# georgeretsi/smirk

Measured on NVIDIA H100. Metric: faces/sec encode->FLAME->render @224^2, higher is better.
Workload: dtype tf32x3

## Files before the change

smirk_b200/csrc/xdw_tc.cu:

```cuda
#include "gemm_tc.cuh"
#include "xdw_tc.cuh"
#include "tc_ptx.cuh"

namespace smk {
namespace {

constexpr int BKB = 128, BK = 32, MMA_K = 8;
constexpr int WIN = 16;
constexpr int HALF_BYTES = 128 * BKB;
constexpr int KB_BYTES = 2 * HALF_BYTES;
constexpr int NC = 32;
constexpr int B_BYTES = NC * BKB;
constexpr int E_PITCH = NC + 4;
constexpr int E_FLOATS = 256 * E_PITCH, E_BYTES = E_FLOATS * 4;
constexpr int PAR_ROWS = 13;
constexpr int PAR_FLOATS = PAR_ROWS * NC, PAR_SLOT_BYTES = PAR_FLOATS * 4;
constexpr int NUM_WORKERS = 256;
constexpr int NUM_THREADS = NUM_WORKERS + 32;
constexpr int DW_THREADS = 128, DW_ROLES = NUM_WORKERS / DW_THREADS, WS_THREADS = NUM_WORKERS + DW_THREADS + 128;
constexpr int WS_LAUNCH_REGS = 65536 / WS_THREADS, MMA_REGS = 168, DW_REGS = 136, PROD_REGS = 40;
static_assert(NUM_WORKERS * MMA_REGS + DW_THREADS * DW_REGS + 128 * PROD_REGS == 65536, "register budgets of the pipelined schedule");
static_assert(MMA_REGS >= WS_LAUNCH_REGS && DW_REGS >= WS_LAUNCH_REGS && PROD_REGS <= WS_LAUNCH_REGS,
              "setmaxnreg directions: inc for the MMA and depthwise warpgroups, dec for the producer");
constexpr int MAX_NKB = 5;
constexpr int SMEM_PER_SM = 228 * 1024, SMEM_PER_CTA = 227 * 1024, SMEM_RESERVED = 1024;

template <int NKB, int X3> struct XdwSmem {
    static constexpr int WIN_BYTES = NKB * KB_BYTES;
    static constexpr int STAGE_BYTES = X3 ? 2 * B_BYTES : B_BYTES;
    static constexpr size_t bytes(int wbuf, int stages, int ne) {
        return (size_t)wbuf * WIN_BYTES + stages * STAGE_BYTES + ne * E_BYTES + (X3 ? ne : 2) * PAR_SLOT_BYTES + 256 + 1024;
    }
    static constexpr bool fits(int wbuf, int stages, int ne, int minb) {
        return bytes(wbuf, stages, ne) <= SMEM_PER_CTA && minb * (bytes(wbuf, stages, ne) + SMEM_RESERVED) <= SMEM_PER_SM;
    }
    static constexpr int MINB = !X3 && fits(1, 2, 1, 2) ? 2 : 1;
    static constexpr int NE = X3 && fits(1, 2, 2, 1) ? 2 : 1;
    static constexpr int STAGES = NKB > 2 && fits(1, NKB, NE, MINB) ? NKB : 2;
    static constexpr int WBUF = fits(2, STAGES, NE, MINB) ? 2 : 1;
    static constexpr size_t SMEM = bytes(WBUF, STAGES, NE);
    static constexpr int RING = WBUF * WIN_BYTES, E_OFF = RING + STAGES * STAGE_BYTES, PAR_OFF = E_OFF + NE * E_BYTES,
                         BAR_OFF = PAR_OFF + (X3 ? NE : 2) * PAR_SLOT_BYTES;
    static_assert(fits(WBUF, STAGES, NE, MINB), "shared-memory budget");
    static_assert(2 * (STAGES + WBUF + NE) * 8 <= 256, "barrier block");
};
static_assert(XdwSmem<1, 2>::NE == 2 && XdwSmem<2, 2>::NE == 2 && XdwSmem<3, 2>::NE == 2 && XdwSmem<4, 2>::NE == 2,
              "3xTF32: two E slots for every window the encoder launches (Cin <= 112)");

using namespace ptx;
__device__ __forceinline__ void worker_barrier() { named_barrier(1, NUM_WORKERS); }

struct XdwMaps { CUtensorMap x[2], w[2], wlo[2]; };

struct XdwArgs {
    int H, W, Ho, Wo;
    int mid, nchunks;
    int groups, chunks_per_group;
    int n_items, B;
    int d_grp, d_tx, d_ty, d_img;
    unsigned geom;
    int pad;
    int tiles_x, tiles_y;
    const float* scale1[2]; const float* bias1[2];
    const float* wdw[2];
    const float* scale2[2]; const float* bias2[2];
    float* out[2];
    int round_out;
    float* e_out[2];
};

struct Item { int prob, img, oh0, ow0, c_begin, c_end; };
struct ItemIter {
    int item, grp, tx, ty, img2;
    __device__ explicit ItemIter(const XdwArgs& a) {
        int v = item = blockIdx.x;
        grp = v % a.groups; v /= a.groups; tx = v % a.tiles_x; v /= a.tiles_x; ty = v % a.tiles_y; img2 = v / a.tiles_y;
    }
    __device__ void next(const XdwArgs& a) {
        item += gridDim.x;
        grp += a.d_grp; if (grp >= a.groups) { grp -= a.groups; ++tx; }
        tx += a.d_tx;   if (tx >= a.tiles_x) { tx -= a.tiles_x; ++ty; }
        ty += a.d_ty;   if (ty >= a.tiles_y) { ty -= a.tiles_y; ++img2; }
        img2 += a.d_img;
    }
    template <int TO> __device__ Item decode(const XdwArgs& a) const {
        Item w;
        w.prob = img2 >= a.B ? 1 : 0; w.img = img2 - w.prob * a.B;
        w.oh0 = ty * TO; w.ow0 = tx * TO;
        w.c_begin = grp * a.chunks_per_group; w.c_end = min(a.nchunks, w.c_begin + a.chunks_per_group);
        return w;
    }
};

template <int STRIDE, int X3, int NKB>
__device__ __forceinline__ void produce(const XdwMaps& mp, const XdwArgs& a, uint8_t* smem, uint64_t* full, uint64_t* empty,
                                        uint64_t* wfull, uint64_t* wempty) {
    using L = XdwSmem<NKB, X3>;
    constexpr int TO = STRIDE == 1 ? 14 : 7, STAGES = L::STAGES, WBUF = L::WBUF;
    uint8_t* ring = smem + L::RING;
    int it = 0, n = 0;
    for (ItemIter ii(a); ii.item < a.n_items; ii.next(a), ++n) {
        const Item w = ii.decode<TO>(a);
        const int ey0 = w.oh0 * STRIDE - a.pad, ex0 = w.ow0 * STRIDE - a.pad;
        const int b = n % WBUF;
        mbar_wait(&wempty[b], ((uint32_t)(n / WBUF) & 1u) ^ 1u);
        uint8_t* win = smem + b * L::WIN_BYTES;
        mbar_expect_tx(&wfull[b], (uint32_t)L::WIN_BYTES);
#pragma unroll
        for (int kb = 0; kb < NKB; ++kb) {
            tma_load_4d(&mp.x[w.prob], win + kb * KB_BYTES, &wfull[b], kb * BK, ex0, ey0, w.img);
            tma_load_4d(&mp.x[w.prob], win + kb * KB_BYTES + HALF_BYTES, &wfull[b], kb * BK, ex0, ey0 + 8, w.img);
        }
        for (int c = w.c_begin; c < w.c_end; ++c)
            for (int kb = 0; kb < NKB; ++kb, ++it) {
                const int s = it % STAGES;
                mbar_wait(&empty[s], ((uint32_t)(it / STAGES) & 1u) ^ 1u);
                uint8_t* st = ring + s * L::STAGE_BYTES;
                mbar_expect_tx(&full[s], (uint32_t)L::STAGE_BYTES);
                tma_load_2d(&mp.w[w.prob], st, &full[s], kb * BK, c * NC);
                if (X3) tma_load_2d(&mp.wlo[w.prob], st + B_BYTES, &full[s], kb * BK, c * NC);
            }
    }
}

struct ParLoader {
    const float* src[2];
    int prow, pcol;
    bool owner;
    __device__ ParLoader(const XdwArgs& a, int t) : src{nullptr, nullptr}, prow(t >> 4), pcol((t & 15) * 2), owner(t < PAR_ROWS * 16) {
        if (owner) {
#pragma unroll
            for (int q = 0; q < 2; ++q)
                src[q] = (prow == 0 ? a.scale1[q] : prow == 1 ? a.bias1[q] : prow == 11 ? a.scale2[q] : prow == 12 ? a.bias2[q]
                                                                                  : a.wdw[q] + (size_t)(prow - 2) * a.mid) + pcol;
        }
    }
    __device__ float2 load(const XdwArgs& a, int prob, int c) const {
        float2 v = make_float2(0.f, 0.f);
        if (owner && c * NC + pcol < a.mid) v = __ldg(reinterpret_cast<const float2*>(src[prob] + c * NC));
        return v;
    }
    __device__ void park(float* par, const float2& v) const {
        if (owner) *reinterpret_cast<float2*>(par + prow * NC + pcol) = v;
    }
};

template <int X3, int NKB, int KSL>
__device__ __forceinline__ void expand_gemm(float (&acc)[2][NC / 2], const uint8_t* win, uint8_t* ring, uint64_t* full, uint64_t* empty,
                                            int& it, int wq, int lane) {
    using L = XdwSmem<NKB, X3>;
    constexpr int STAGES = L::STAGES;
#pragma unroll
    for (int mb = 0; mb < 2; ++mb)
#pragma unroll
        for (int i = 0; i < NC / 2; ++i) acc[mb][i] = 0.f;
#pragma unroll
    for (int kb = 0; kb < NKB; ++kb, ++it) {
        const int nks = kb + 1 < NKB ? BK / MMA_K : KSL;
        const int s = it % STAGES;
        mbar_wait(&full[s], (uint32_t)(it / STAGES) & 1u);
        const uint8_t* xa = win + kb * KB_BYTES;
        const uint32_t sb = smem_u32(ring + s * L::STAGE_BYTES);
        if constexpr (X3 != 0) {
            uint32_t hi[2][BK / MMA_K][4], lo[2][BK / MMA_K][4];
#pragma unroll
            for (int mb = 0; mb < 2; ++mb)
#pragma unroll
                for (int k = 0; k < nks; ++k) {
                    float v[4];
                    load_a_frag(xa, mb * 64, k * MMA_K, wq, lane, v);
                    split_frag(v, hi[mb][k], lo[mb][k]);
                }
            wgmma_fence();
#pragma unroll
            for (int k = 0; k < nks; ++k) {
                const uint64_t db = make_smem_desc(sb + k * MMA_K * 4);
                const uint64_t dbl = make_smem_desc(sb + B_BYTES + k * MMA_K * 4);
#pragma unroll
                for (int mb = 0; mb < 2; ++mb) {
                    Wgmma<NC>::rs(acc[mb], hi[mb][k], db, 1u);
                    Wgmma<NC>::rs(acc[mb], lo[mb][k], db, 1u);
                    Wgmma<NC>::rs(acc[mb], hi[mb][k], dbl, 1u);
                }
            }
        } else {
            const uint32_t sa = smem_u32(xa);
            wgmma_fence();
#pragma unroll
            for (int k = 0; k < nks; ++k) {
                const uint64_t db = make_smem_desc(sb + k * MMA_K * 4);
#pragma unroll
                for (int mb = 0; mb < 2; ++mb)
                    Wgmma<NC>::ss(acc[mb], make_smem_desc(sa + mb * 64 * BKB + k * MMA_K * 4), db, 1u);
            }
        }
        wgmma_commit();
        wgmma_wait<0>();
        __syncwarp();
        mbar_arrive_if(&empty[s], lane == 0);
    }
}

template <int STRIDE, bool SAVE>
__device__ __forceinline__ void bn1_relu(const float (&acc)[2][NC / 2], float* E, const float* par, const XdwArgs& a, const Item& w,
                                         int ch0, int half, int wq, int lane) {
    constexpr int TO = STRIDE == 1 ? 14 : 7;
    const int ey0 = w.oh0 * STRIDE - a.pad, ex0 = w.ow0 * STRIDE - a.pad;
#pragma unroll
    for (int mb = 0; mb < 2; ++mb)
#pragma unroll
        for (int hr = 0; hr < 2; ++hr) {
            const int r = mb * 64 + wq * 16 + (lane >> 2) + 8 * hr;
            const int ey = ey0 + half * 8 + (r >> 4), ex = ex0 + (r & 15);
            const bool inside = ey >= 0 && ey < a.H && ex >= 0 && ex < a.W;
            float* erow = E + (size_t)(half * 128 + r) * E_PITCH;
            bool own = false;
            float* esave = nullptr;
            if constexpr (SAVE) {
                own = inside && ey >= w.oh0 * STRIDE && ey < (w.oh0 + TO) * STRIDE && ex >= w.ow0 * STRIDE && ex < (w.ow0 + TO) * STRIDE;
                esave = a.e_out[w.prob] + (((size_t)w.img * a.H + ey) * a.W + ex) * a.mid + ch0;
            }
#pragma unroll
            for (int j = 0; j < NC / 8; ++j) {
                const int ch = 8 * j + 2 * (lane & 3);
                float2 o = make_float2(0.f, 0.f);
                if (inside) {
                    const float2 sc = *reinterpret_cast<const float2*>(par + ch);
                    const float2 bi = *reinterpret_cast<const float2*>(par + NC + ch);
                    o.x = fmaxf(fmaf(acc[mb][4 * j + 2 * hr], sc.x, bi.x), 0.f);
                    o.y = fmaxf(fmaf(acc[mb][4 * j + 2 * hr + 1], sc.y, bi.y), 0.f);
                }
                *reinterpret_cast<float2*>(erow + ch) = o;
                if (SAVE && own && ch0 + ch < a.mid) *reinterpret_cast<float2*>(esave + ch) = o;
            }
        }
}

template <int TO> __device__ __forceinline__ unsigned dw_role(const XdwArgs& a, int slot) {
    const int ncols_e = a.Wo - (a.tiles_x - 1) * TO;
    return (unsigned)(slot % TO) | (unsigned)(slot / TO) << 8 | (unsigned)(slot % ncols_e) << 16 | (unsigned)(slot / ncols_e) << 24;
}
struct DwRows { int ox, oy0, oy1; };
template <int TO> __device__ __forceinline__ DwRows dw_rows(const XdwArgs& a, const ItemIter& ii, unsigned role) {
    const bool col_e = ii.tx == a.tiles_x - 1, row_e = ii.ty == a.tiles_y - 1;
    const int nrows = row_e ? a.Ho - (a.tiles_y - 1) * TO : TO;
    const unsigned g8 = a.geom >> ((col_e ? 16 : 0) + (row_e ? 8 : 0));
    const int rpt = (int)(g8 & 15u), n_rg = (int)((g8 >> 4) & 15u);
    const unsigned r16 = role >> (col_e ? 16 : 0);
    const int rg = (int)((r16 >> 8) & 255u);
    DwRows d;
    d.ox = (int)(r16 & 255u); d.oy0 = rg * rpt; d.oy1 = rg < n_rg ? min(nrows, d.oy0 + rpt) : 0;
    return d;
}

template <int STRIDE>
__device__ __forceinline__ void depthwise(const float* E, const float* par, const XdwArgs& a, const Item& w, int ch0, int cq, const DwRows& rows) {
    if (cq * 4 < a.mid - ch0 && rows.oy0 < rows.oy1) {
        const int ch = ch0 + cq * 4;
        float4 k[9];
#pragma unroll
        for (int q = 0; q < 9; ++q) k[q] = *reinterpret_cast<const float4*>(par + (2 + q) * NC + cq * 4);
        const float4 s2 = *reinterpret_cast<const float4*>(par + 11 * NC + cq * 4);
        const float4 b2 = *reinterpret_cast<const float4*>(par + 12 * NC + cq * 4);
        float* orow = a.out[w.prob] + (((size_t)w.img * a.Ho + w.oh0 + rows.oy0) * a.Wo + w.ow0 + rows.ox) * a.mid + ch;
        const size_t orow_stride = (size_t)a.Wo * a.mid;
        auto emit = [&](const float4& acc4) {
            float4 o = fma4(acc4, s2, b2);
            o.x = fmaxf(o.x, 0.f); o.y = fmaxf(o.y, 0.f); o.z = fmaxf(o.z, 0.f); o.w = fmaxf(o.w, 0.f);
            if (a.round_out) { o.x = round_tf32(o.x); o.y = round_tf32(o.y); o.z = round_tf32(o.z); o.w = round_tf32(o.w); }
            *reinterpret_cast<float4*>(orow) = o;
            orow += orow_stride;
        };
        const float* e = E + (size_t)((rows.oy0 * STRIDE) * WIN + rows.ox * STRIDE) * E_PITCH + cq * 4;
        const float4 zero = make_float4(0.f, 0.f, 0.f, 0.f);
        if (STRIDE == 1) {
            float4 acc0 = zero, acc1 = zero, acc2 = zero;
            const int n_in = rows.oy1 - rows.oy0 + 2;
#pragma unroll 3
            for (int r = 0; r < n_in; ++r, e += WIN * E_PITCH) {
                const float4 x0 = *reinterpret_cast<const float4*>(e);
                const float4 x1 = *reinterpret_cast<const float4*>(e + E_PITCH);
                const float4 x2 = *reinterpret_cast<const float4*>(e + 2 * E_PITCH);
                fma4_acc(acc0, x0, k[6]); fma4_acc(acc0, x1, k[7]); fma4_acc(acc0, x2, k[8]);
                fma4_acc(acc1, x0, k[3]); fma4_acc(acc1, x1, k[4]); fma4_acc(acc1, x2, k[5]);
                fma4_acc(acc2, x0, k[0]); fma4_acc(acc2, x1, k[1]); fma4_acc(acc2, x2, k[2]);
                if (r >= 2) emit(acc0);
                acc0 = acc1; acc1 = acc2; acc2 = zero;
            }
        } else {
            float4 p0 = *reinterpret_cast<const float4*>(e);
            float4 p1 = *reinterpret_cast<const float4*>(e + E_PITCH);
            float4 p2 = *reinterpret_cast<const float4*>(e + 2 * E_PITCH);
            for (int oy = rows.oy0; oy < rows.oy1; ++oy) {
                e += WIN * E_PITCH;
                float4 acc4 = zero;
                fma4_acc(acc4, p0, k[0]); fma4_acc(acc4, p1, k[1]); fma4_acc(acc4, p2, k[2]);
                const float4 m0 = *reinterpret_cast<const float4*>(e);
                const float4 m1 = *reinterpret_cast<const float4*>(e + E_PITCH);
                const float4 m2 = *reinterpret_cast<const float4*>(e + 2 * E_PITCH);
                fma4_acc(acc4, m0, k[3]); fma4_acc(acc4, m1, k[4]); fma4_acc(acc4, m2, k[5]);
                e += WIN * E_PITCH;
                p0 = *reinterpret_cast<const float4*>(e);
                p1 = *reinterpret_cast<const float4*>(e + E_PITCH);
                p2 = *reinterpret_cast<const float4*>(e + 2 * E_PITCH);
                fma4_acc(acc4, p0, k[6]); fma4_acc(acc4, p1, k[7]); fma4_acc(acc4, p2, k[8]);
                emit(acc4);
            }
        }
    }
}

template <int NKB, int X3> struct XdwShared {
    using L = XdwSmem<NKB, X3>;
    uint8_t* smem;
    float* E;
    float* PAR;
    uint64_t *full, *empty;
    uint64_t *wfull, *wempty;
    uint64_t *efull, *eempty;
    __device__ explicit XdwShared(uint8_t* raw) {
        smem = raw + ((1024u - (smem_u32(raw) & 1023u)) & 1023u);
        E = reinterpret_cast<float*>(smem + L::E_OFF);
        PAR = reinterpret_cast<float*>(smem + L::PAR_OFF);
        full = reinterpret_cast<uint64_t*>(smem + L::BAR_OFF);
        empty = full + L::STAGES;
        wfull = empty + L::STAGES;
        wempty = wfull + L::WBUF;
        efull = wempty + L::WBUF;
        eempty = efull + L::NE;
    }
};

template <int STRIDE, int X3, int NKB, int KSL, bool SAVE>
__global__ void __launch_bounds__(NUM_THREADS, XdwSmem<NKB, X3>::MINB)
xdw_kernel(const __grid_constant__ XdwMaps mp, const XdwArgs a) {
    using L = XdwSmem<NKB, X3>;
    constexpr int TO = STRIDE == 1 ? 14 : 7;
    extern __shared__ uint8_t smem_raw[];
    const XdwShared<NKB, X3> sh(smem_raw);
    const int warp = threadIdx.x >> 5, lane = threadIdx.x & 31;
    if (warp == NUM_WORKERS / 32 && lane == 0) {
        prefetch_tensormap(&mp.x[0]);
        prefetch_tensormap(&mp.w[0]);
        for (int s = 0; s < L::STAGES; ++s) { mbar_init(&sh.full[s], 1); mbar_init(&sh.empty[s], NUM_WORKERS / 32); }
        for (int b = 0; b < L::WBUF; ++b) { mbar_init(&sh.wfull[b], 1); mbar_init(&sh.wempty[b], NUM_WORKERS / 32); }
        fence_barrier_init();
    }
    __syncthreads();

    if (warp == NUM_WORKERS / 32) {
        if (lane == 0) produce<STRIDE, X3, NKB>(mp, a, sh.smem, sh.full, sh.empty, sh.wfull, sh.wempty);
        return;
    }

    const int half = warp >> 2, wq = warp & 3;
    const int t = threadIdx.x;
    const int cq = t & 7;
    const ParLoader pl(a, t);
    ItemIter ii(a);
    if (ii.item < a.n_items) { const Item w0 = ii.decode<TO>(a); pl.park(sh.PAR, pl.load(a, w0.prob, w0.c_begin)); }
    worker_barrier();
    const unsigned role = dw_role<TO>(a, t >> 3);
    int cc = 0, it = 0;
    for (int n = 0; ii.item < a.n_items; ++n) {
      const Item w = ii.decode<TO>(a);
      const int wb = n % L::WBUF;
      const uint8_t* win = sh.smem + wb * L::WIN_BYTES + half * HALF_BYTES;
      mbar_wait(&sh.wfull[wb], (uint32_t)(n / L::WBUF) & 1u);
      const DwRows rows = dw_rows<TO>(a, ii, role);
      int next_first = -1, next_prob = 0;
      ii.next(a);
      if (ii.item < a.n_items) { const Item wn = ii.decode<TO>(a); next_first = wn.c_begin; next_prob = wn.prob; }
      for (int c = w.c_begin; c < w.c_end; ++c, ++cc) {
        const int buf = cc & 1;
        const float* par = sh.PAR + buf * PAR_FLOATS;
        const int c_next = c + 1 < w.c_end ? c + 1 : next_first;
        float2 pf = make_float2(0.f, 0.f);
        if (c_next >= 0) pf = pl.load(a, c + 1 < w.c_end ? w.prob : next_prob, c_next);
        float acc[2][NC / 2];
        expand_gemm<X3, NKB, KSL>(acc, win, sh.smem + L::RING, sh.full, sh.empty, it, wq, lane);
        mbar_arrive_if(&sh.wempty[wb], lane == 0 && c + 1 == w.c_end);
        bn1_relu<STRIDE, SAVE>(acc, sh.E, par, a, w, c * NC, half, wq, lane);
        if (c_next >= 0) pl.park(sh.PAR + (buf ^ 1) * PAR_FLOATS, pf);
        worker_barrier();
        depthwise<STRIDE>(sh.E, par, a, w, c * NC, cq, rows);
        worker_barrier();
      }
    }
}

template <int STRIDE, int X3, int NKB, int KSL, bool SAVE>
__global__ void __launch_bounds__(WS_THREADS, 1)
xdw_ws_kernel(const __grid_constant__ XdwMaps mp, const XdwArgs a) {
    using L = XdwSmem<NKB, X3>;
    constexpr int TO = STRIDE == 1 ? 14 : 7, NE = L::NE;
    constexpr int PROD_WARP = (NUM_WORKERS + DW_THREADS) / 32;
    extern __shared__ uint8_t smem_raw[];
    const XdwShared<NKB, X3> sh(smem_raw);
    const int warp = threadIdx.x >> 5, lane = threadIdx.x & 31;
    if (warp == PROD_WARP && lane == 0) {
        prefetch_tensormap(&mp.x[0]);
        prefetch_tensormap(&mp.w[0]);
        prefetch_tensormap(&mp.wlo[0]);
        for (int s = 0; s < L::STAGES; ++s) { mbar_init(&sh.full[s], 1); mbar_init(&sh.empty[s], NUM_WORKERS / 32); }
        for (int b = 0; b < L::WBUF; ++b) { mbar_init(&sh.wfull[b], 1); mbar_init(&sh.wempty[b], NUM_WORKERS / 32); }
        for (int s = 0; s < NE; ++s) { mbar_init(&sh.efull[s], NUM_WORKERS); mbar_init(&sh.eempty[s], DW_THREADS); }
        fence_barrier_init();
    }
    __syncthreads();

    if (warp >= PROD_WARP) {
        setmaxnreg_dec<PROD_REGS>();
        if (warp == PROD_WARP && lane == 0) produce<STRIDE, X3, NKB>(mp, a, sh.smem, sh.full, sh.empty, sh.wfull, sh.wempty);
        return;
    }

    if (warp >= NUM_WORKERS / 32) {
        setmaxnreg_inc<DW_REGS>();
        const int d = threadIdx.x - NUM_WORKERS, cq = d & 7;
        unsigned role[DW_ROLES];
#pragma unroll
        for (int j = 0; j < DW_ROLES; ++j) role[j] = dw_role<TO>(a, (d >> 3) + j * (DW_THREADS / 8));
        int cc = 0;
        for (ItemIter ii(a); ii.item < a.n_items; ii.next(a)) {
            const Item w = ii.decode<TO>(a);
            DwRows rows[DW_ROLES];
#pragma unroll
            for (int j = 0; j < DW_ROLES; ++j) rows[j] = dw_rows<TO>(a, ii, role[j]);
            for (int c = w.c_begin; c < w.c_end; ++c, ++cc) {
                const int s = cc % NE;
                mbar_wait(&sh.efull[s], (uint32_t)(cc / NE) & 1u);
#pragma unroll 1
                for (int j = 0; j < DW_ROLES; ++j) depthwise<STRIDE>(sh.E + s * E_FLOATS, sh.PAR + s * PAR_FLOATS, a, w, c * NC, cq, rows[j]);
                mbar_arrive(&sh.eempty[s]);
            }
        }
        return;
    }

    setmaxnreg_inc<MMA_REGS>();
    const int half = warp >> 2, wq = warp & 3;
    const ParLoader pl(a, threadIdx.x);
    int cc = 0, it = 0, n = 0;
    for (ItemIter ii(a); ii.item < a.n_items; ii.next(a), ++n) {
        const Item w = ii.decode<TO>(a);
        const int wb = n % L::WBUF;
        const uint8_t* win = sh.smem + wb * L::WIN_BYTES + half * HALF_BYTES;
        mbar_wait(&sh.wfull[wb], (uint32_t)(n / L::WBUF) & 1u);
        for (int c = w.c_begin; c < w.c_end; ++c, ++cc) {
            const int s = cc % NE;
            float* par = sh.PAR + s * PAR_FLOATS;
            const float2 pf = pl.load(a, w.prob, c);
            float acc[2][NC / 2];
            expand_gemm<X3, NKB, KSL>(acc, win, sh.smem + L::RING, sh.full, sh.empty, it, wq, lane);
            mbar_arrive_if(&sh.wempty[wb], lane == 0 && c + 1 == w.c_end);
            mbar_wait(&sh.eempty[s], ((uint32_t)(cc / NE) & 1u) ^ 1u);
            pl.park(par, pf);
            worker_barrier();
            bn1_relu<STRIDE, SAVE>(acc, sh.E + s * E_FLOATS, par, a, w, c * NC, half, wq, lane);
            mbar_arrive(&sh.efull[s]);
        }
    }
}

template <int STRIDE, int X3, int NKB, int KSL, bool SAVE>
int launch(const XdwMaps& mp, const XdwArgs& a, int grid, cudaStream_t st) {
    constexpr size_t smem = XdwSmem<NKB, X3>::SMEM;
    if constexpr (X3 != 0) {
        SMK_CHECK_CUDA((set_max_dynamic_smem<xdw_ws_kernel<STRIDE, X3, NKB, KSL, SAVE>>((int)smem)));
        SMK_LAUNCH((xdw_ws_kernel<STRIDE, X3, NKB, KSL, SAVE>), dim3(grid), dim3(WS_THREADS), smem, st, mp, a);
    } else {
        SMK_CHECK_CUDA((set_max_dynamic_smem<xdw_kernel<STRIDE, X3, NKB, KSL, SAVE>>((int)smem)));
        SMK_LAUNCH((xdw_kernel<STRIDE, X3, NKB, KSL, SAVE>), dim3(grid), dim3(NUM_THREADS), smem, st, mp, a);
    }
    SMK_CHECK_LAUNCH();
    return 0;
}

template <int STRIDE, int X3, int NKB, int KSL>
int launch_save(const XdwMaps& mp, const XdwArgs& a, int grid, cudaStream_t st) {
    return a.e_out[0] ? launch<STRIDE, X3, NKB, KSL, true>(mp, a, grid, st) : launch<STRIDE, X3, NKB, KSL, false>(mp, a, grid, st);
}

template <int STRIDE, int X3, int NKB>
int launch_ksl(int ksl, const XdwMaps& mp, const XdwArgs& a, int grid, cudaStream_t st) {
    switch (ksl) {
        case 1: return launch_save<STRIDE, X3, NKB, 1>(mp, a, grid, st);
        case 2: return launch_save<STRIDE, X3, NKB, 2>(mp, a, grid, st);
        case 3: return launch_save<STRIDE, X3, NKB, 3>(mp, a, grid, st);
        default: return launch_save<STRIDE, X3, NKB, 4>(mp, a, grid, st);
    }
}

template <int STRIDE, int X3>
int launch_cin(int Cin, const XdwMaps& mp, const XdwArgs& a, int grid, cudaStream_t st) {
    static_assert(MAX_NKB == 5, "one case per window size");
    const int nkb = cdiv(Cin, BK), ksl = cdiv(Cin, MMA_K) - (nkb - 1) * (BK / MMA_K);
    switch (nkb) {
        case 1: return launch_ksl<STRIDE, X3, 1>(ksl, mp, a, grid, st);
        case 2: return launch_ksl<STRIDE, X3, 2>(ksl, mp, a, grid, st);
        case 3: return launch_ksl<STRIDE, X3, 3>(ksl, mp, a, grid, st);
        case 4: return launch_ksl<STRIDE, X3, 4>(ksl, mp, a, grid, st);
        default: return launch_ksl<STRIDE, X3, 5>(ksl, mp, a, grid, st);
    }
}

}

int xdw_conv(const XdwConv& p, cudaStream_t st, const XdwConv* p2) {
    const int nprob = p2 ? 2 : 1;
    SMK_REQUIRE(p.stride == 1 || p.stride == 2, "xdw_conv: stride must be 1 or 2");
    SMK_REQUIRE(p.Cin % 4 == 0 && p.mid % 4 == 0, "xdw_conv: Cin and mid must be multiples of 4");
    SMK_REQUIRE(p.Cin > 0 && p.Cin <= MAX_NKB * BK, "xdw_conv: Cin must be at most 160 (the whole input window stays in shared memory)");
    SMK_REQUIRE(p.stride == 1 || (p.H % 2 == 0 && p.W % 2 == 0), "xdw_conv: stride 2 expects even input sizes (TF-SAME pad_begin 0)");
    SMK_REQUIRE(!p2 || (p2->B == p.B && p2->H == p.H && p2->W == p.W && p2->Cin == p.Cin && p2->mid == p.mid && p2->stride == p.stride &&
                        p2->round_out == p.round_out && !p2->w1t_lo == !p.w1t_lo && !p2->e_out == !p.e_out),
                "xdw_conv: paired problems must have identical shapes");
    const int Ho = (p.H + p.stride - 1) / p.stride, Wo = (p.W + p.stride - 1) / p.stride;
    const int TO = p.stride == 1 ? 14 : 7;
    XdwMaps mp;
    XdwArgs a{};
    for (int g = 0; g < nprob; ++g) {
        const XdwConv& q = g ? *p2 : p;
        if (int rc = encode_nhwc(&mp.x[g], q.x, q.B, q.H, q.W, q.Cin, q.Cin, WIN, 8, "xdw_conv(x)")) return rc;
        if (int rc = encode_2d(&mp.w[g], q.w1t, (uint64_t)q.mid, (uint64_t)q.Cin, (uint64_t)q.Cin, NC, "xdw_conv(w1)")) return rc;
        mp.wlo[g] = mp.w[g];
        if (q.w1t_lo) { if (int rc = encode_2d(&mp.wlo[g], q.w1t_lo, (uint64_t)q.mid, (uint64_t)q.Cin, (uint64_t)q.Cin, NC, "xdw_conv(w1 tails)")) return rc; }
        a.scale1[g] = q.scale1; a.bias1[g] = q.bias1; a.wdw[g] = q.wdw; a.scale2[g] = q.scale2; a.bias2[g] = q.bias2; a.out[g] = q.out;
        a.e_out[g] = q.e_out;
    }
    if (nprob == 1) {
        mp.x[1] = mp.x[0]; mp.w[1] = mp.w[0]; mp.wlo[1] = mp.wlo[0];
        a.scale1[1] = a.scale1[0]; a.bias1[1] = a.bias1[0]; a.wdw[1] = a.wdw[0]; a.scale2[1] = a.scale2[0]; a.bias2[1] = a.bias2[0]; a.out[1] = a.out[0];
        a.e_out[1] = a.e_out[0];
    }
    const int slots = num_sms();
    a.H = p.H; a.W = p.W; a.Ho = Ho; a.Wo = Wo; a.mid = p.mid; a.nchunks = cdiv(p.mid, NC);
    {
        const long tiles = (long)nprob * cdiv(Wo, TO) * cdiv(Ho, TO) * p.B;
        int groups = (int)std::min<long>(a.nchunks, std::max<long>(1, (slots + tiles - 1) / tiles));
        a.chunks_per_group = cdiv(a.nchunks, groups);
        a.groups = cdiv(a.nchunks, a.chunks_per_group);
    }
    a.pad = p.stride == 1 ? 1 : 0;
    a.tiles_x = cdiv(Wo, TO); a.tiles_y = cdiv(Ho, TO);
    a.round_out = p.round_out;
    {
        const double px_in = (double)nprob * p.B * p.H * p.W, px_out = (double)nprob * p.B * Ho * Wo;
        const char* tag = p.w1t_lo ? "xdw_fused_tc3x" : "xdw_fused_tc";
        if (g_prof_detail) tag = prof_shape_tag(tag, (long)px_out, p.Cin, p.mid);
        SMK_TAG(tag, 4.0 * (px_in * p.Cin + px_out * p.mid + (double)nprob * p.mid * (p.Cin + 13)), 2.0 * px_in * p.Cin * p.mid + 18.0 * px_out * p.mid, st);
    }
    a.B = p.B;
    a.n_items = nprob * a.tiles_x * a.tiles_y * p.B * a.groups;
    {
        const int ncols_e = Wo - (a.tiles_x - 1) * TO, nrows_e = Ho - (a.tiles_y - 1) * TO;
        auto group = [](int ncols, int nrows) { const int n_rg = std::min(32 / ncols, nrows); return (unsigned)((nrows + n_rg - 1) / n_rg) | (unsigned)n_rg << 4; };
        a.geom = group(TO, TO) | group(TO, nrows_e) << 8 | group(ncols_e, TO) << 16 | group(ncols_e, nrows_e) << 24;
    }
    const int grid = std::min(a.n_items, slots);
    { int v = grid; a.d_grp = v % a.groups; v /= a.groups; a.d_tx = v % a.tiles_x; v /= a.tiles_x; a.d_ty = v % a.tiles_y; a.d_img = v / a.tiles_y; }
    if (p.w1t_lo) return p.stride == 1 ? launch_cin<1, 2>(p.Cin, mp, a, grid, st) : launch_cin<2, 2>(p.Cin, mp, a, grid, st);
    return p.stride == 1 ? launch_cin<1, 0>(p.Cin, mp, a, grid, st) : launch_cin<2, 0>(p.Cin, mp, a, grid, st);
}

}

extern "C" int smk_debug_xdw(const float* x, int B, int H, int W, int Cin, const float* w1t, const float* scale1, const float* bias1,
                             int mid, const float* wdw, const float* scale2, const float* bias2, int stride, int round_out,
                             float* out, void* stream) {
    smk::XdwConv p{};
    p.x = x; p.B = B; p.H = H; p.W = W; p.Cin = Cin; p.w1t = w1t; p.scale1 = scale1; p.bias1 = bias1; p.mid = mid; p.wdw = wdw;
    p.scale2 = scale2; p.bias2 = bias2; p.stride = stride; p.round_out = round_out; p.out = out;
    return smk::xdw_conv(p, (cudaStream_t)stream);
}

extern "C" int smk_debug_xdw3x(const float* x, int B, int H, int W, int Cin, const float* w1t_hi, const float* w1t_lo, const float* scale1,
                               const float* bias1, int mid, const float* wdw, const float* scale2, const float* bias2, int stride,
                               float* out, void* stream) {
    smk::XdwConv p{};
    p.x = x; p.B = B; p.H = H; p.W = W; p.Cin = Cin; p.w1t = w1t_hi; p.w1t_lo = w1t_lo; p.scale1 = scale1; p.bias1 = bias1; p.mid = mid; p.wdw = wdw;
    p.scale2 = scale2; p.bias2 = bias2; p.stride = stride; p.round_out = 0; p.out = out;
    return smk::xdw_conv(p, (cudaStream_t)stream);
}
```

Measured before the change: 26320.

## Move BN param staging to depthwise warpgroup and compute two columns per role

```diff
diff --git a/smirk_b200/csrc/xdw_tc.cu b/smirk_b200/csrc/xdw_tc.cu
--- a/smirk_b200/csrc/xdw_tc.cu
+++ b/smirk_b200/csrc/xdw_tc.cu
@@ -17,7 +17,7 @@
 constexpr int PAR_FLOATS = PAR_ROWS * NC, PAR_SLOT_BYTES = PAR_FLOATS * 4;
 constexpr int NUM_WORKERS = 256;
 constexpr int NUM_THREADS = NUM_WORKERS + 32;
-constexpr int DW_THREADS = 128, DW_ROLES = NUM_WORKERS / DW_THREADS, WS_THREADS = NUM_WORKERS + DW_THREADS + 128;
+constexpr int DW_THREADS = 128, WS_THREADS = NUM_WORKERS + DW_THREADS + 128;
 constexpr int WS_LAUNCH_REGS = 65536 / WS_THREADS, MMA_REGS = 168, DW_REGS = 136, PROD_REGS = 40;
 static_assert(NUM_WORKERS * MMA_REGS + DW_THREADS * DW_REGS + 128 * PROD_REGS == 65536, "register budgets of the pipelined schedule");
 static_assert(MMA_REGS >= WS_LAUNCH_REGS && DW_REGS >= WS_LAUNCH_REGS && PROD_REGS <= WS_LAUNCH_REGS,
@@ -29,7 +29,7 @@
     static constexpr int WIN_BYTES = NKB * KB_BYTES;
     static constexpr int STAGE_BYTES = X3 ? 2 * B_BYTES : B_BYTES;
     static constexpr size_t bytes(int wbuf, int stages, int ne) {
-        return (size_t)wbuf * WIN_BYTES + stages * STAGE_BYTES + ne * E_BYTES + (X3 ? ne : 2) * PAR_SLOT_BYTES + 256 + 1024;
+        return (size_t)wbuf * WIN_BYTES + stages * STAGE_BYTES + ne * E_BYTES + (X3 ? 2 * ne : 2) * PAR_SLOT_BYTES + 256 + 1024;
     }
     static constexpr bool fits(int wbuf, int stages, int ne, int minb) {
         return bytes(wbuf, stages, ne) <= SMEM_PER_CTA && minb * (bytes(wbuf, stages, ne) + SMEM_RESERVED) <= SMEM_PER_SM;
@@ -40,7 +40,7 @@
     static constexpr int WBUF = fits(2, STAGES, NE, MINB) ? 2 : 1;
     static constexpr size_t SMEM = bytes(WBUF, STAGES, NE);
     static constexpr int RING = WBUF * WIN_BYTES, E_OFF = RING + STAGES * STAGE_BYTES, PAR_OFF = E_OFF + NE * E_BYTES,
-                         BAR_OFF = PAR_OFF + (X3 ? NE : 2) * PAR_SLOT_BYTES;
+                         BAR_OFF = PAR_OFF + (X3 ? 2 * NE : 2) * PAR_SLOT_BYTES;
     static_assert(fits(WBUF, STAGES, NE, MINB), "shared-memory budget");
     static_assert(2 * (STAGES + WBUF + NE) * 8 <= 256, "barrier block");
 };
@@ -91,6 +91,18 @@
         return w;
     }
 };
+template <int TO> struct ChunkIter {
+    ItemIter ii;
+    int prob, c, c_end;
+    __device__ explicit ChunkIter(const XdwArgs& a) : ii(a) { start(a); }
+    __device__ bool valid(const XdwArgs& a) const { return ii.item < a.n_items; }
+    __device__ void start(const XdwArgs& a) {
+        if (valid(a)) { const Item w = ii.decode<TO>(a); prob = w.prob; c = w.c_begin; c_end = w.c_end; }
+    }
+    __device__ void next(const XdwArgs& a) {
+        if (valid(a) && ++c == c_end) { ii.next(a); start(a); }
+    }
+};
 
 template <int STRIDE, int X3, int NKB>
 __device__ __forceinline__ void produce(const XdwMaps& mp, const XdwArgs& a, uint8_t* smem, uint64_t* full, uint64_t* empty,
@@ -135,9 +147,9 @@
                                                                                   : a.wdw[q] + (size_t)(prow - 2) * a.mid) + pcol;
         }
     }
-    __device__ float2 load(const XdwArgs& a, int prob, int c) const {
+    template <bool SELECT = false> __device__ float2 load(const XdwArgs& a, int prob, int c) const {
         float2 v = make_float2(0.f, 0.f);
-        if (owner && c * NC + pcol < a.mid) v = __ldg(reinterpret_cast<const float2*>(src[prob] + c * NC));
+        if (owner && c * NC + pcol < a.mid) v = __ldg(reinterpret_cast<const float2*>((SELECT ? (prob ? src[1] : src[0]) : src[prob]) + c * NC));
         return v;
     }
     __device__ void park(float* par, const float2& v) const {
@@ -236,25 +248,30 @@
         }
 }
 
-template <int TO> __device__ __forceinline__ unsigned dw_role(const XdwArgs& a, int slot) {
-    const int ncols_e = a.Wo - (a.tiles_x - 1) * TO;
-    return (unsigned)(slot % TO) | (unsigned)(slot / TO) << 8 | (unsigned)(slot % ncols_e) << 16 | (unsigned)(slot / ncols_e) << 24;
-}
-struct DwRows { int ox, oy0, oy1; };
-template <int TO> __device__ __forceinline__ DwRows dw_rows(const XdwArgs& a, const ItemIter& ii, unsigned role) {
+__host__ __device__ constexpr int dw_cols(int stride, bool pipelined) { return stride == 1 && pipelined ? 2 : 1; }
+template <int STRIDE, int DWC> __device__ __forceinline__ unsigned dw_role(const XdwArgs& a, int slot) {
+    constexpr int TO = STRIDE == 1 ? 14 : 7, NCR = (TO + DWC - 1) / DWC;
+    const int ncr_e = (a.Wo - (a.tiles_x - 1) * TO + DWC - 1) / DWC;
+    return (unsigned)(slot % NCR * DWC) | (unsigned)(slot / NCR) << 8 | (unsigned)(slot % ncr_e * DWC) << 16 | (unsigned)(slot / ncr_e) << 24;
+}
+struct DwRows { int ox, ncol, oy0, oy1; };
+template <int STRIDE, int DWC> __device__ __forceinline__ DwRows dw_rows(const XdwArgs& a, const ItemIter& ii, unsigned role) {
+    constexpr int TO = STRIDE == 1 ? 14 : 7;
     const bool col_e = ii.tx == a.tiles_x - 1, row_e = ii.ty == a.tiles_y - 1;
-    const int nrows = row_e ? a.Ho - (a.tiles_y - 1) * TO : TO;
+    const int nrows = row_e ? a.Ho - (a.tiles_y - 1) * TO : TO, ncols = col_e ? a.Wo - (a.tiles_x - 1) * TO : TO;
     const unsigned g8 = a.geom >> ((col_e ? 16 : 0) + (row_e ? 8 : 0));
     const int rpt = (int)(g8 & 15u), n_rg = (int)((g8 >> 4) & 15u);
     const unsigned r16 = role >> (col_e ? 16 : 0);
     const int rg = (int)((r16 >> 8) & 255u);
     DwRows d;
-    d.ox = (int)(r16 & 255u); d.oy0 = rg * rpt; d.oy1 = rg < n_rg ? min(nrows, d.oy0 + rpt) : 0;
+    d.ox = (int)(r16 & 255u); d.ncol = min(DWC, ncols - d.ox);
+    d.oy0 = rg * rpt; d.oy1 = rg < n_rg ? min(nrows, d.oy0 + rpt) : 0;
     return d;
 }
 
-template <int STRIDE>
+template <int STRIDE, int DWC>
 __device__ __forceinline__ void depthwise(const float* E, const float* par, const XdwArgs& a, const Item& w, int ch0, int cq, const DwRows& rows) {
+    static_assert(STRIDE == 1 || DWC == 1, "stride 2 runs one column per role");
     if (cq * 4 < a.mid - ch0 && rows.oy0 < rows.oy1) {
         const int ch = ch0 + cq * 4;
         float4 k[9];
@@ -264,16 +281,19 @@
         const float4 b2 = *reinterpret_cast<const float4*>(par + 12 * NC + cq * 4);
         float* orow = a.out[w.prob] + (((size_t)w.img * a.Ho + w.oh0 + rows.oy0) * a.Wo + w.ow0 + rows.ox) * a.mid + ch;
         const size_t orow_stride = (size_t)a.Wo * a.mid;
-        auto emit = [&](const float4& acc4) {
+        auto bn2 = [&](const float4& acc4) {
             float4 o = fma4(acc4, s2, b2);
             o.x = fmaxf(o.x, 0.f); o.y = fmaxf(o.y, 0.f); o.z = fmaxf(o.z, 0.f); o.w = fmaxf(o.w, 0.f);
             if (a.round_out) { o.x = round_tf32(o.x); o.y = round_tf32(o.y); o.z = round_tf32(o.z); o.w = round_tf32(o.w); }
-            *reinterpret_cast<float4*>(orow) = o;
+            return o;
+        };
+        auto emit = [&](const float4& acc4) {
+            *reinterpret_cast<float4*>(orow) = bn2(acc4);
             orow += orow_stride;
         };
         const float* e = E + (size_t)((rows.oy0 * STRIDE) * WIN + rows.ox * STRIDE) * E_PITCH + cq * 4;
         const float4 zero = make_float4(0.f, 0.f, 0.f, 0.f);
-        if (STRIDE == 1) {
+        if (STRIDE == 1 && DWC == 1) {
             float4 acc0 = zero, acc1 = zero, acc2 = zero;
             const int n_in = rows.oy1 - rows.oy0 + 2;
 #pragma unroll 3
@@ -287,6 +307,45 @@
                 if (r >= 2) emit(acc0);
                 acc0 = acc1; acc1 = acc2; acc2 = zero;
             }
+        } else if (STRIDE == 1) {
+            struct Acc { float4 c[DWC]; };
+            float4 x[DWC + 2];
+            auto load = [&](int r) {
+#pragma unroll
+                for (int j = 0; j < DWC + 2; ++j) x[j] = *reinterpret_cast<const float4*>(e + (r * WIN + j) * E_PITCH);
+            };
+            auto fresh = [&]() {
+                Acc acc;
+#pragma unroll
+                for (int j = 0; j < DWC; ++j) acc.c[j] = zero;
+                return acc;
+            };
+            auto taps = [&](Acc& acc, int ky) {
+#pragma unroll
+                for (int kx = 0; kx < 3; ++kx)
+#pragma unroll
+                    for (int j = 0; j < DWC; ++j) fma4_acc(acc.c[j], x[kx + j], k[3 * ky + kx]);
+            };
+            auto store = [&](const Acc& acc) {
+#pragma unroll
+                for (int j = 0; j < DWC; ++j)
+                    if (j == 0 || j < rows.ncol) *reinterpret_cast<float4*>(orow + j * a.mid) = bn2(acc.c[j]);
+                orow += orow_stride;
+            };
+            const int n_out = rows.oy1 - rows.oy0;
+            Acc p, q = fresh();
+            load(0); taps(q, 0);
+            load(1); p = q; taps(p, 1);
+            if (n_out > 1) { q = fresh(); taps(q, 0); }
+#pragma unroll 2
+            for (int r = 2; r < n_out; ++r) {
+                load(r);
+                taps(p, 2); store(p);
+                p = q; taps(p, 1);
+                q = fresh(); taps(q, 0);
+            }
+            if (n_out > 1) { load(n_out); taps(p, 2); store(p); p = q; taps(p, 1); }
+            load(n_out + 1); taps(p, 2); store(p);
         } else {
             float4 p0 = *reinterpret_cast<const float4*>(e);
             float4 p1 = *reinterpret_cast<const float4*>(e + E_PITCH);
@@ -360,14 +419,15 @@
     ItemIter ii(a);
     if (ii.item < a.n_items) { const Item w0 = ii.decode<TO>(a); pl.park(sh.PAR, pl.load(a, w0.prob, w0.c_begin)); }
     worker_barrier();
-    const unsigned role = dw_role<TO>(a, t >> 3);
+    constexpr int DWC = dw_cols(STRIDE, false);
+    const unsigned role = dw_role<STRIDE, DWC>(a, t >> 3);
     int cc = 0, it = 0;
     for (int n = 0; ii.item < a.n_items; ++n) {
       const Item w = ii.decode<TO>(a);
       const int wb = n % L::WBUF;
       const uint8_t* win = sh.smem + wb * L::WIN_BYTES + half * HALF_BYTES;
       mbar_wait(&sh.wfull[wb], (uint32_t)(n / L::WBUF) & 1u);
-      const DwRows rows = dw_rows<TO>(a, ii, role);
+      const DwRows rows = dw_rows<STRIDE, DWC>(a, ii, role);
       int next_first = -1, next_prob = 0;
       ii.next(a);
       if (ii.item < a.n_items) { const Item wn = ii.decode<TO>(a); next_first = wn.c_begin; next_prob = wn.prob; }
@@ -383,7 +443,7 @@
         bn1_relu<STRIDE, SAVE>(acc, sh.E, par, a, w, c * NC, half, wq, lane);
         if (c_next >= 0) pl.park(sh.PAR + (buf ^ 1) * PAR_FLOATS, pf);
         worker_barrier();
-        depthwise<STRIDE>(sh.E, par, a, w, c * NC, cq, rows);
+        depthwise<STRIDE, DWC>(sh.E, par, a, w, c * NC, cq, rows);
         worker_barrier();
       }
     }
@@ -418,20 +478,32 @@
     if (warp >= NUM_WORKERS / 32) {
         setmaxnreg_inc<DW_REGS>();
         const int d = threadIdx.x - NUM_WORKERS, cq = d & 7;
-        unsigned role[DW_ROLES];
-#pragma unroll
-        for (int j = 0; j < DW_ROLES; ++j) role[j] = dw_role<TO>(a, (d >> 3) + j * (DW_THREADS / 8));
+        constexpr int DWC = dw_cols(STRIDE, true);
+        const unsigned role = dw_role<STRIDE, DWC>(a, d >> 3);
+        const ParLoader pl0(a, d), pl1(a, d + DW_THREADS);
+        ChunkIter<TO> ahead(a);
+        for (int j = 0; j < NE; ++j, ahead.next(a)) {
+            if (ahead.valid(a)) {
+                float* par = sh.PAR + j * PAR_FLOATS;
+                pl0.park(par, pl0.load<true>(a, ahead.prob, ahead.c)); pl1.park(par, pl1.load<true>(a, ahead.prob, ahead.c));
+            }
+            mbar_arrive(&sh.eempty[j]);
+        }
         int cc = 0;
         for (ItemIter ii(a); ii.item < a.n_items; ii.next(a)) {
             const Item w = ii.decode<TO>(a);
-            DwRows rows[DW_ROLES];
-#pragma unroll
-            for (int j = 0; j < DW_ROLES; ++j) rows[j] = dw_rows<TO>(a, ii, role[j]);
-            for (int c = w.c_begin; c < w.c_end; ++c, ++cc) {
+            const DwRows rows = dw_rows<STRIDE, DWC>(a, ii, role);
+            for (int c = w.c_begin; c < w.c_end; ++c, ++cc, ahead.next(a)) {
                 const int s = cc % NE;
+                const bool stage = ahead.valid(a);
+                float2 pf0 = make_float2(0.f, 0.f), pf1 = pf0;
+                if (stage) { pf0 = pl0.load<true>(a, ahead.prob, ahead.c); pf1 = pl1.load<true>(a, ahead.prob, ahead.c); }
                 mbar_wait(&sh.efull[s], (uint32_t)(cc / NE) & 1u);
-#pragma unroll 1
-                for (int j = 0; j < DW_ROLES; ++j) depthwise<STRIDE>(sh.E + s * E_FLOATS, sh.PAR + s * PAR_FLOATS, a, w, c * NC, cq, rows[j]);
+                depthwise<STRIDE, DWC>(sh.E + s * E_FLOATS, sh.PAR + (cc % (2 * NE)) * PAR_FLOATS, a, w, c * NC, cq, rows);
+                if (stage) {
+                    float* par = sh.PAR + ((cc + NE) % (2 * NE)) * PAR_FLOATS;
+                    pl0.park(par, pf0); pl1.park(par, pf1);
+                }
                 mbar_arrive(&sh.eempty[s]);
             }
         }
@@ -440,7 +512,6 @@
 
     setmaxnreg_inc<MMA_REGS>();
     const int half = warp >> 2, wq = warp & 3;
-    const ParLoader pl(a, threadIdx.x);
     int cc = 0, it = 0, n = 0;
     for (ItemIter ii(a); ii.item < a.n_items; ii.next(a), ++n) {
         const Item w = ii.decode<TO>(a);
@@ -449,15 +520,11 @@
         mbar_wait(&sh.wfull[wb], (uint32_t)(n / L::WBUF) & 1u);
         for (int c = w.c_begin; c < w.c_end; ++c, ++cc) {
             const int s = cc % NE;
-            float* par = sh.PAR + s * PAR_FLOATS;
-            const float2 pf = pl.load(a, w.prob, c);
             float acc[2][NC / 2];
             expand_gemm<X3, NKB, KSL>(acc, win, sh.smem + L::RING, sh.full, sh.empty, it, wq, lane);
             mbar_arrive_if(&sh.wempty[wb], lane == 0 && c + 1 == w.c_end);
-            mbar_wait(&sh.eempty[s], ((uint32_t)(cc / NE) & 1u) ^ 1u);
-            pl.park(par, pf);
-            worker_barrier();
-            bn1_relu<STRIDE, SAVE>(acc, sh.E + s * E_FLOATS, par, a, w, c * NC, half, wq, lane);
+            mbar_wait(&sh.eempty[s], (uint32_t)(cc / NE) & 1u);
+            bn1_relu<STRIDE, SAVE>(acc, sh.E + s * E_FLOATS, sh.PAR + (cc % (2 * NE)) * PAR_FLOATS, a, w, c * NC, half, wq, lane);
             mbar_arrive(&sh.efull[s]);
         }
     }
@@ -555,7 +622,11 @@
     a.n_items = nprob * a.tiles_x * a.tiles_y * p.B * a.groups;
     {
         const int ncols_e = Wo - (a.tiles_x - 1) * TO, nrows_e = Ho - (a.tiles_y - 1) * TO;
-        auto group = [](int ncols, int nrows) { const int n_rg = std::min(32 / ncols, nrows); return (unsigned)((nrows + n_rg - 1) / n_rg) | (unsigned)n_rg << 4; };
+        const int dw_slots = (p.w1t_lo ? DW_THREADS : NUM_WORKERS) / (NC / 4), dwc = dw_cols(p.stride, p.w1t_lo != nullptr);
+        auto group = [&](int ncols, int nrows) {
+            const int n_rg = std::min(dw_slots / cdiv(ncols, dwc), nrows);
+            return (unsigned)cdiv(nrows, n_rg) | (unsigned)n_rg << 4;
+        };
         a.geom = group(TO, TO) | group(TO, nrows_e) << 8 | group(ncols_e, TO) << 16 | group(ncols_e, nrows_e) << 24;
     }
     const int grid = std::min(a.n_items, slots);
```

Result: faster. 27880, median of 6 (+5.9%).
